# gchq/annchor

Hardware: AMD Instinct MI355X
Metric: knn_graph_builds_per_s (1 / Annchor.fit() wall-clock; BASELINE: k-NN graph build time + recall@k) (higher is better)
Workload: dtype int32 bit-vectors (Levenshtein) + f64 (bounds/regression/selection); 1 GPU; load_strings Levenshtein N=1600 n_anchors=15 k=25 p_work=0.12 niters=2; parallelism=one GPU

## Files before the change

annchor_amd/csrc/ctx.hip:

```cpp
#include <cstdarg>
#include <cmath>
#include <cstdlib>

#include "common.h"
#include <algorithm>
#include <chrono>
#include <mutex>

static std::string g_create_err;
void ann_stream_release(annchor_ctx *c);
void ann_enemies_release(annchor_ctx *c);
void ann_draw_forget(annchor_ctx *c);
void ann_comm_release(annchor_ctx *c);
hipError_t ann_comm_guarded_sync(annchor_ctx *c, hipStream_t stream, const char *where);

const char *ann_set_err(annchor_ctx *c, const char *fmt, ...)
{
    char buf[1024];
    va_list ap;
    va_start(ap, fmt);
    vsnprintf(buf, sizeof buf, fmt, ap);
    va_end(ap);
    if (c && c->comm_aborted && c->err.rfind("collective timed out", 0) == 0) return c->err.c_str();
    if (c) c->err = buf; else g_create_err = buf;
// ... 179 lines not shown
        ANN_CHECK_HIP(c, hipMemcpyAsync(dst, slot, bytes, hipMemcpyHostToDevice, c->stream));
        ANN_CHECK_HIP(c, hipEventRecord(c->pin_ev[sl], c->stream));
        c->pin_busy[sl] = true;
        return ANNCHOR_OK;
    }
    ANN_CHECK_HIP(c, hipMemcpyAsync(dst, src, bytes, hipMemcpyHostToDevice, c->stream));
    ANN_CHECK_HIP(c, ann_sync(c, __func__));
    return ANNCHOR_OK;
}

hipError_t ann_sync(annchor_ctx *c, const char *where)
{
    static const bool trace = getenv("ANNCHOR_SYNC_TRACE") != nullptr;
    static const bool timing = getenv("ANNCHOR_SYNC_TIMING") != nullptr;
    if (trace) fprintf(stderr, "sync %s\n", where);
    const long long t_in = timing ? ann_now_ns() : 0;
    if (c->idle_gen_n > c->idle_gen_done) {
        c->idle_gen_done = std::min(c->idle_gen_n, c->idle_gen_done + c->idle_gen_chunk);
        (void)ann_legacy_generate_upto(c->idle_gen_seed, c->idle_gen_n, c->idle_gen_done);
    }
    const long long t_w = timing ? ann_now_ns() : 0;
    if (c->side_pending) (void)ann_side_join(c);
    const hipError_t rc = c->comm ? ann_comm_guarded_sync(c, c->stream, where) : hipStreamSynchronize(c->stream);
    if (timing) fprintf(stderr, "T wait %s %lld %lld %lld\n", where, t_in, t_w, ann_now_ns());
    if (c->lev_ap_probe_epoch) ann_lev_ap_probe(c);
    return rc;
}

extern "C" int annchor_legacy_generate_at_next_wait(annchor_ctx *c, uint32_t seed, int64_t ndraws, int64_t chunk)
{
    if (!c || ndraws < 0) return ANNCHOR_EINVAL;
    c->idle_gen_seed = seed;
    c->idle_gen_n = ndraws;
    c->idle_gen_done = 0;
    c->idle_gen_chunk = chunk > 0 ? chunk : ndraws;
    return ANNCHOR_OK;
}

int ann_d2h(annchor_ctx *c, void *dst, const void *src, size_t bytes)
{
    if (bytes == 0) return ANNCHOR_OK;
    if (c->pin && bytes <= annchor_ctx::PIN_DL_BYTES) {
        unsigned char *slot = c->pin + (size_t)annchor_ctx::PIN_SLOTS * annchor_ctx::PIN_SLOT_BYTES;
        ANN_CHECK_HIP(c, hipMemcpyAsync(slot, src, bytes, hipMemcpyDeviceToHost, c->stream));
        ANN_CHECK_HIP(c, ann_sync(c, __func__));
        memcpy(dst, slot, bytes);
        return ANNCHOR_OK;
    }
    ANN_CHECK_HIP(c, hipMemcpyAsync(dst, src, bytes, hipMemcpyDeviceToHost, c->stream));
    ANN_CHECK_HIP(c, ann_sync(c, __func__));
    return ANNCHOR_OK;
}

int ann_d2h2(annchor_ctx *c, void *dst1, const void *src1, size_t bytes1, void *dst2, const void *src2, size_t bytes2)
{
    const size_t off2 = (bytes1 + 63) & ~(size_t)63;
    if (c->pin && off2 + bytes2 <= annchor_ctx::PIN_DL_BYTES) {
        unsigned char *slot = c->pin + (size_t)annchor_ctx::PIN_SLOTS * annchor_ctx::PIN_SLOT_BYTES;
        ANN_CHECK_HIP(c, hipMemcpyAsync(slot, src1, bytes1, hipMemcpyDeviceToHost, c->stream));
        ANN_CHECK_HIP(c, hipMemcpyAsync(slot + off2, src2, bytes2, hipMemcpyDeviceToHost, c->stream));
        ANN_CHECK_HIP(c, ann_sync(c, __func__));
        memcpy(dst1, slot, bytes1);
        memcpy(dst2, slot + off2, bytes2);
        return ANNCHOR_OK;
    }
    ANN_TRY(ann_d2h(c, dst1, src1, bytes1));
    return ann_d2h(c, dst2, src2, bytes2);
}

int ann_d2h_then(annchor_ctx *c, void *dst, const void *src, size_t bytes, int (*then)(annchor_ctx *))
{
    if (!c->pin || bytes > annchor_ctx::PIN_DL_BYTES) {
        ANN_TRY(ann_d2h(c, dst, src, bytes));
        return then(c);
    }
    if (!c->dl_ev) ANN_CHECK_HIP(c, hipEventCreate(&c->dl_ev));
    unsigned char *slot = c->pin + (size_t)annchor_ctx::PIN_SLOTS * annchor_ctx::PIN_SLOT_BYTES;
    ANN_CHECK_HIP(c, hipMemcpyAsync(slot, src, bytes, hipMemcpyDeviceToHost, c->stream));
    ANN_CHECK_HIP(c, hipEventRecord(c->dl_ev, c->stream));
    const int rc = then(c);
    static const bool trace = getenv("ANNCHOR_SYNC_TRACE") != nullptr;
    static const bool timing = getenv("ANNCHOR_SYNC_TIMING") != nullptr;
    if (trace) fprintf(stderr, "sync %s\n", __func__);
    const long long t_w = timing ? ann_now_ns() : 0;
    ANN_CHECK_HIP(c, hipEventSynchronize(c->dl_ev));
    if (timing) fprintf(stderr, "T wait %s %lld %lld %lld\n", __func__, t_w, t_w, ann_now_ns());
    memcpy(dst, slot, bytes);
    return rc;
}

int ann_prof_entry(annchor_ctx *c, const char *name)
{
    for (size_t i = 0; i < c->prof.size(); ++i)
        if (c->prof[i].name == name || strcmp(c->prof[i].name, name) == 0) return (int)i;
    ProfEntry e;
    e.name = name;
    c->prof.push_back(e);
    return (int)c->prof.size() - 1;
}

static void prof_drain(annchor_ctx *c)
{
    for (auto &p : c->pending) {
        float ms = 0;
        if (hipEventSynchronize(p.b) == hipSuccess && hipEventElapsedTime(&ms, p.a, p.b) == hipSuccess)
            c->prof[p.entry].ms += ms;
        c->ev_pool.push_back(p.a);
        c->ev_pool.push_back(p.b);
    }
    c->pending.clear();
}

ProfScope::ProfScope(annchor_ctx *ctx, const char *name, double alg_bytes) : c(ctx)
{
    if (!c->prof_on) return;
    if (c->prof_mode == 2) {
        const size_t n = strlen(name);
        if (n < 6 || strcmp(name + n - 6, "_pairs") != 0) return;
    }
    entry = ann_prof_entry(c, name);
    c->prof[entry].launches += 1;
    c->prof[entry].alg_bytes += alg_bytes;
    if (entry == c->prof_group_entry) { entry = -1; return; }
    auto get = [&](hipEvent_t *e) {
        if (!c->ev_pool.empty()) { *e = c->ev_pool.back(); c->ev_pool.pop_back(); return true; }
        return hipEventCreate(e) == hipSuccess;
    };
    if (!get(&a) || !get(&b)) { entry = -1; return; }
    (void)hipEventRecord(a, c->stream);
}

ProfGroup::ProfGroup(annchor_ctx *ctx, const char *name) : c(ctx)
{
    if (!c->prof_on || c->prof_group_entry >= 0) return;
    if (c->prof_mode == 2) {
        const size_t n = strlen(name);
        if (n < 6 || strcmp(name + n - 6, "_pairs") != 0) return;
    }
    entry = ann_prof_entry(c, name);
    auto get = [&](hipEvent_t *e) {
        if (!c->ev_pool.empty()) { *e = c->ev_pool.back(); c->ev_pool.pop_back(); return true; }
        return hipEventCreate(e) == hipSuccess;
    };
    if (!get(&a) || !get(&b)) { entry = -1; return; }
    (void)hipEventRecord(a, c->stream);
    c->prof_group_entry = entry;
}

ProfGroup::~ProfGroup()
{
    if (entry < 0) return;
    (void)hipEventRecord(b, c->stream);
    c->pending.push_back({entry, a, b});
    c->prof_group_entry = -1;
}

ProfScope::~ProfScope()
{
    if (entry < 0) return;
    (void)hipEventRecord(b, c->stream);
    c->pending.push_back({entry, a, b});
    if (c->pending.size() > 4096) prof_drain(c);
}

extern "C" int annchor_prof_enable(annchor_ctx *c, int32_t on)
{
    if (!c) return ANNCHOR_EINVAL;
    c->prof_on = on != 0;
    c->prof_mode = on;
    return ANNCHOR_OK;
// ... 1073 lines not shown
```

annchor_amd/csrc/locality.hip:

```cpp
#include "common.h"

template <int NW> __global__ void k_sid(const double *__restrict__ Dt, int64_t nx, int na, int locality, uint64_t *__restrict__ sid,
                                        int32_t *__restrict__ cA)
{
    int64_t i = (int64_t)blockIdx.x * blockDim.x + threadIdx.x;
    if (i >= nx) return;
    Sid<NW> mask = sid_zero<NW>();
    int first = 0;
    for (int r = 0; r < locality; ++r) {
        double best = INFINITY;
        int ba = -1;
        for (int a = 0; a < na; ++a) {
            if ((mask.w[NW == 1 ? 0 : a >> 6] >> (a & 63)) & 1ull) continue;
            double v = Dt[(size_t)a * nx + i];
            if (ba < 0 || v < best) { best = v; ba = a; }
        }
        if (ba < 0) break;
        if (r == 0) first = ba;
#pragma unroll
        for (int w = 0; w < NW; ++w)
            if (w == (ba >> 6)) mask.w[w] |= 1ull << (ba & 63);
    }
#pragma unroll
    for (int w = 0; w < NW; ++w) sid[i * NW + w] = mask.w[w];
    cA[i] = first;
}

#define LOC_THREADS 256
template <int NW>
__global__ __launch_bounds__(LOC_THREADS) void k_loc_thresh(const uint64_t *__restrict__ sid, int64_t nx, int loc_thresh,
                                                           int loc_min, int32_t *__restrict__ thr)
{
    __shared__ uint32_t hist[ANN_MASK_ANCHORS + 1];
    for (int t = threadIdx.x; t < ANN_MASK_ANCHORS + 1; t += blockDim.x) hist[t] = 0;
    __syncthreads();
    const int64_t i = blockIdx.x;
    const Sid<NW> mi = sid_ld<NW>(sid, i);
    for (int64_t j = threadIdx.x; j < nx; j += blockDim.x) atomicAdd(&hist[sid_common<NW>(mi, sid_ld<NW>(sid, j))], 1u);
    __syncthreads();
    if (threadIdx.x == 0) {
        int64_t lm = loc_min < nx - 1 ? loc_min : nx - 1;
        int64_t cum = 0;
        int v = ANN_MASK_ANCHORS;
        for (; v >= 0; --v) {
            cum += hist[v];
            if (cum >= lm + 1) break;
        }
        if (v < 0) v = 0;
        thr[i] = v < loc_thresh ? v : loc_thresh;
    }
}

template <int T, int NW>
__global__ __launch_bounds__(LOC_THREADS) void k_loc_thresh_small(const uint64_t *__restrict__ sid, int64_t nx, int loc_min, int32_t *__restrict__ thr)
{
    __shared__ uint32_t part[LOC_THREADS / 64][T];
    const int64_t i = blockIdx.x;
    const Sid<NW> mi = sid_ld<NW>(sid, i);
    uint32_t c[T];
#pragma unroll
    for (int t = 0; t < T; ++t) c[t] = 0;
    for (int64_t j0 = threadIdx.x; j0 < nx; j0 += 4 * LOC_THREADS) {
        Sid<NW> mj[4];
#pragma unroll
        for (int e = 0; e < 4; ++e) mj[e] = sid_ld<NW>(sid, min(j0 + e * LOC_THREADS, nx - 1));
#pragma unroll
        for (int e = 0; e < 4; ++e) {
            const int cc = j0 + e * LOC_THREADS < nx ? sid_common<NW>(mi, mj[e]) : 0;
#pragma unroll
            for (int t = 0; t < T; ++t) c[t] += cc > t;
        }
    }
#pragma unroll
    for (int t = 0; t < T; ++t) {
#pragma unroll
        for (int off = 32; off > 0; off >>= 1) c[t] += __shfl_xor(c[t], off);
    }
    if ((threadIdx.x & 63) == 0)
#pragma unroll
        for (int t = 0; t < T; ++t) part[threadIdx.x >> 6][t] = c[t];
    __syncthreads();
    if (threadIdx.x == 0) {
        const int64_t lm = loc_min < nx - 1 ? loc_min : nx - 1;
        int v = 0;
#pragma unroll
        for (int t = 0; t < T; ++t) {
            uint32_t g = 0;
            for (int w = 0; w < LOC_THREADS / 64; ++w) g += part[w][t];
            if ((int64_t)g >= lm + 1) v = t + 1;
        }
        thr[i] = v;
    }
}

template <int NW>
__global__ __launch_bounds__(256) void k_keep_bits(const uint64_t *__restrict__ sid, const int32_t *__restrict__ thr, int64_t nx, int kw,
                                                  uint64_t *__restrict__ K)
{
    const int lane = threadIdx.x & 63;
    const int64_t wave_global = ((int64_t)blockIdx.x * blockDim.x + threadIdx.x) >> 6;
    const int64_t wave_count = ((int64_t)gridDim.x * blockDim.x) >> 6;
    const int64_t items = nx * kw;
    const int64_t per = (items + wave_count - 1) / wave_count;
    const int64_t t0 = wave_global * per, t1 = min(t0 + per, items);
    for (int64_t t = t0; t < t1; ++t) {
        const int64_t i = t / kw;
        const int w = (int)(t - i * kw);
        const Sid<NW> mi = sid_ld<NW>(sid, i);
        const int ti = thr[i];
        const int64_t j = (int64_t)w * 64 + lane;
        bool keep = false;
        if (j < nx && j != i) {
            const int cc = sid_common<NW>(mi, sid_ld<NW>(sid, j));
            const int tj = thr[j];
            keep = cc >= (ti < tj ? ti : tj);
        }
        const unsigned long long bits = __ballot(keep);
        if (lane == 0) K[t] = bits;
    }
}

template <int NW>
__global__ __launch_bounds__(256) void k_keep_bits_cols(const uint64_t *__restrict__ sid, const int32_t *__restrict__ thr, int64_t nx, int kw,
                                                       uint64_t *__restrict__ K)
{
    const int lane = threadIdx.x & 63;
    const int wave = __builtin_amdgcn_readfirstlane((int)(threadIdx.x >> 6));
    const int64_t task = (int64_t)blockIdx.x * 4 + wave;
    const int64_t rb = task / kw;
    const int w = (int)(task - rb * kw);
    if (rb * 64 >= nx) return;
    const int64_t i0 = rb * 64, i_base = min(i0, nx - 64);
    const int64_t j = (int64_t)w * 64 + lane;
    const bool jv = j < nx;
    const Sid<NW> mj = jv ? sid_ld<NW>(sid, j) : sid_zero<NW>();
    const int tj = jv ? thr[j] : 0;
    int r_lo = 0, r_hi = 0;
#pragma unroll 16
    for (int r = 0; r < 64; ++r) {
        const int64_t i = i_base + r;
        const Sid<NW> mi = sid_ld<NW>(sid, i);
        const int ti = thr[i];
        const int cc = sid_common<NW>(mi, mj);
        const bool keep = jv && j != i && cc >= (ti < tj ? ti : tj);
        const unsigned long long bits = __ballot(keep);
        r_lo = lane == r ? (int)(uint32_t)bits : r_lo;
        r_hi = lane == r ? (int)(uint32_t)(bits >> 32) : r_hi;
    }
    const int64_t i = i_base + lane;
    if (i >= i0) K[i * kw + w] = ((uint64_t)(uint32_t)r_hi << 32) | (uint32_t)r_lo;
}

__global__ void k_sid_wide(const double *__restrict__ Dt, int64_t nx, int na, int L, int nw, int kw, uint64_t *__restrict__ sid,
                           uint16_t *__restrict__ sidl, uint64_t *__restrict__ sidm, int32_t *__restrict__ cA)
{
    const int64_t i = (int64_t)blockIdx.x * blockDim.x + threadIdx.x;
    if (i >= nx) return;
    double pv = -INFINITY;
    int pa = -1, first = 0;
    for (int r = 0; r < L; ++r) {
        double best = INFINITY;
        int ba = -1;
        for (int a = 0; a < na; ++a) {
            const double v = Dt[(size_t)a * nx + i];
            const bool after = v > pv || (v == pv && a > pa);
            if (after && (ba < 0 || v < best)) { best = v; ba = a; }
        }
        if (ba < 0) {
            for (; r < L; ++r) sidl[i * L + r] = 0xffff;
            break;
        }
        if (r == 0) first = ba;
        sidl[i * L + r] = (uint16_t)ba;
        sid[i * nw + (ba >> 6)] |= 1ull << (ba & 63);
        atomicOr(reinterpret_cast<unsigned long long *>(sidm) + (size_t)ba * kw + (i >> 6), 1ull << (i & 63));
        pv = best; pa = ba;
    }
    cA[i] = first;
}

template <int T>
__global__ __launch_bounds__(LOC_THREADS) void k_loc_thresh_small_wide(const uint16_t *__restrict__ sidl, const uint64_t *__restrict__ sidm,
                                                                      int L, int na, int kw, int64_t nx, int loc_min, int32_t *__restrict__ thr)
{
    __shared__ uint32_t part[LOC_THREADS / 64][T];
    const int64_t i = blockIdx.x;
    uint32_t c[T];
#pragma unroll
    for (int t = 0; t < T; ++t) c[t] = 0;
    for (int w = threadIdx.x; w < kw; w += LOC_THREADS) {
        uint64_t ge[T + 1];
        ge[0] = ~0ull;
#pragma unroll
        for (int k = 1; k <= T; ++k) ge[k] = 0ull;
        for (int r = 0; r < L; ++r) {
            const int a = sidl[i * L + r];
            const uint64_t m = a < na ? sidm[(size_t)a * kw + w] : 0ull;
#pragma unroll
            for (int k = T; k >= 1; --k) ge[k] |= ge[k - 1] & m;
        }
#pragma unroll
// ... 255 lines not shown
    } else {
        const int64_t t = blockIdx.x;
        jb = (int)((2.0 * nb + 1.0 - sqrt((2.0 * nb + 1.0) * (2.0 * nb + 1.0) - 8.0 * (double)t)) * 0.5);
        while ((int64_t)jb * nb - (int64_t)jb * (jb - 1) / 2 > t) --jb;
        while ((int64_t)(jb + 1) * nb - (int64_t)(jb + 1) * jb / 2 <= t) ++jb;
        ib = jb + (int)(t - ((int64_t)jb * nb - (int64_t)jb * (jb - 1) / 2));
    }
    const int lane = threadIdx.x & 63, wave = threadIdx.x >> 6;
    const int64_t i_r = (int64_t)ib * 64 + lane;
#pragma unroll 4
    for (int q = 0; q < 16; ++q) {
        const int64_t j = (int64_t)jb * 64 + wave * 16 + q;
        int32_t pos = 0;
        if (j < nx) {
            const uint64_t bits = K[j * kw + ib];
            if (i_r > j && ((bits >> lane) & 1ull))
                pos = (int32_t)(rowstart[j] + ((int64_t)pref[j * kw + ib] + __popcll(bits & ((1ull << lane) - 1ull)) - low[j]));
        }
        tp[wave * 16 + q][lane] = pos;
    }
    __syncthreads();
    const int64_t j_w = (int64_t)jb * 64 + lane;
    uint32_t cb_lo = 0, cb_hi = 0, cd_lo = 0, cd_hi = 0;
    {
        const int64_t i = (int64_t)ib * 64 + wave * 16 + (lane & 15);
        if (i < nx) {
            const uint64_t bits = K[i * kw + jb];
            const int64_t dst0 = Iptr[i] + (int64_t)pref[i * kw + jb];
            cb_lo = (uint32_t)bits; cb_hi = (uint32_t)(bits >> 32);
            cd_lo = (uint32_t)dst0; cd_hi = (uint32_t)((uint64_t)dst0 >> 32);
        }
    }
#pragma unroll
    for (int q = 0; q < 16; ++q) {
        const int il = wave * 16 + q;
        const int64_t i = (int64_t)ib * 64 + il;
        const uint64_t bits = ((uint64_t)(uint32_t)__builtin_amdgcn_readlane((int)cb_hi, q) << 32) | (uint32_t)__builtin_amdgcn_readlane((int)cb_lo, q);
        if (j_w < i && ((bits >> lane) & 1ull)) {
            const int64_t dst0 = (int64_t)(((uint64_t)(uint32_t)__builtin_amdgcn_readlane((int)cd_hi, q) << 32) | (uint32_t)__builtin_amdgcn_readlane((int)cd_lo, q));
            ann_store(Iidx + dst0 + __popcll(bits & ((1ull << lane) - 1ull)), tp[lane][il], stream);
        }
    }
}

__global__ void k_min_i32(const int32_t *__restrict__ v, int64_t n, int32_t *__restrict__ out)
{
    int m = 0x7fffffff;
    for (int64_t t = threadIdx.x; t < n; t += blockDim.x) m = min(m, v[t]);
#pragma unroll
    for (int off = 32; off > 0; off >>= 1) m = min(m, __shfl_xor(m, off));
    __shared__ int s[16];
    if ((threadIdx.x & 63) == 0) s[threadIdx.x >> 6] = m;
    __syncthreads();
    if (threadIdx.x == 0) {
        for (int w = 1; w < (int)(blockDim.x >> 6); ++w) m = min(m, s[w]);
        out[0] = m;
        out[1] = 0; out[2] = 0; out[3] = 0;
    }
}

__global__ __launch_bounds__(256) void k_count_anchor_pairs(const int32_t *__restrict__ A, int nA, const int32_t *__restrict__ anchorRank,
                                                           int64_t nx, const uint64_t *__restrict__ K, int kw,
                                                           unsigned long long *__restrict__ out)
{
    const int64_t t = (int64_t)blockIdx.x * blockDim.x + threadIdx.x;
    bool hit = false;
    if (t < (int64_t)nA * nx) {
        const int r = (int)(t / nx);
        const int64_t a = A[r], o = t % nx;
        if (anchorRank[a] == r && a != o && !(anchorRank[o] >= 0 && o < a)) {
            const int64_t i = a < o ? a : o, j = a < o ? o : a;
            hit = (K[i * kw + (j >> 6)] >> (j & 63)) & 1ull;
        }
    }
    const unsigned long long m = __ballot(hit);
    __shared__ uint32_t s;
    if (threadIdx.x == 0) s = 0;
    __syncthreads();
    if ((threadIdx.x & 63) == 0 && m) atomicAdd(&s, (uint32_t)__popcll(m));
    __syncthreads();
    if (threadIdx.x == 0 && s) atomicAdd(out, (unsigned long long)s);
}

static int wide_sets(annchor_ctx *c, int locality)
{
    const int64_t nx = c->nx;
    const int nw = c->sid_nw, kw = (int)((nx + 63) / 64);
    c->sid_L = locality;
    ANN_TRY(ann_reserve(c, c->sidl, sizeof(uint16_t) * (size_t)nx * locality));
    ANN_TRY(ann_reserve(c, c->sidm, sizeof(uint64_t) * (size_t)c->na * kw));
    ANN_CHECK_HIP(c, hipMemsetAsync(c->sid.p, 0, sizeof(uint64_t) * (size_t)nx * nw, c->stream));
    ANN_CHECK_HIP(c, hipMemsetAsync(c->sidm.p, 0, sizeof(uint64_t) * (size_t)c->na * kw, c->stream));
    k_sid_wide<<<ann_blocks(nx, 256), 256, 0, c->stream>>>(c->Dt.as<double>(), nx, c->na, locality, nw, kw, c->sid.as<uint64_t>(),
                                                          c->sidl.as<uint16_t>(), c->sidm.as<uint64_t>(), c->cA.as<int32_t>());
    return ANNCHOR_OK;
}

static int wide_keep_bitmap(annchor_ctx *c, int loc_thresh, int loc_min, int kw)
{
    const int64_t nx = c->nx;
    const int L = c->sid_L, na = c->na;
    const uint16_t *sidl = c->sidl.as<uint16_t>();
    const uint64_t *sidm = c->sidm.as<uint64_t>();
    static const bool hist_form = getenv("ANNCHOR_LOC_THRESH_HIST") != nullptr;
    if (loc_thresh >= 1 && loc_thresh <= 8 && !hist_form) {
        switch (loc_thresh) {
#define LTW_CASE(T) case T: k_loc_thresh_small_wide<T><<<(int)nx, LOC_THREADS, 0, c->stream>>>(sidl, sidm, L, na, kw, nx, loc_min, c->thr.as<int32_t>()); break;
            LTW_CASE(1) LTW_CASE(2) LTW_CASE(3) LTW_CASE(4) LTW_CASE(5) LTW_CASE(6) LTW_CASE(7) LTW_CASE(8)
#undef LTW_CASE
        }
    } else
        k_loc_thresh_wide<<<(int)nx, LOC_THREADS, sizeof(uint32_t) * (size_t)(L + 1), c->stream>>>(sidl, sidm, L, na, kw, nx, loc_thresh,
                                                                                                 loc_min, c->thr.as<int32_t>());
    const unsigned grid = (unsigned)((((nx + 63) / 64) * kw + 3) / 4);
    if (loc_thresh >= 1 && loc_thresh <= 8) {
        switch (loc_thresh) {
#define KBP_CASE(T) case T: k_keep_bits_wide_planes<T><<<grid, 256, 0, c->stream>>>(sidl, sidm, L, na, c->thr.as<int32_t>(), nx, kw, c->Kbits.as<uint64_t>()); break;
            KBP_CASE(1) KBP_CASE(2) KBP_CASE(3) KBP_CASE(4) KBP_CASE(5) KBP_CASE(6) KBP_CASE(7) KBP_CASE(8)
#undef KBP_CASE
        }
        return ANNCHOR_OK;
    }
    switch (L) {
#define KBW_CASE(LC) case LC: k_keep_bits_wide<LC><<<grid, 256, 0, c->stream>>>(sidl, sidm, L, na, c->thr.as<int32_t>(), nx, kw, c->Kbits.as<uint64_t>()); break;
        KBW_CASE(1) KBW_CASE(2) KBW_CASE(3) KBW_CASE(4) KBW_CASE(5) KBW_CASE(6) KBW_CASE(7) KBW_CASE(8)
#undef KBW_CASE
    default: k_keep_bits_wide<0><<<grid, 256, 0, c->stream>>>(sidl, sidm, L, na, c->thr.as<int32_t>(), nx, kw, c->Kbits.as<uint64_t>());
    }
    return ANNCHOR_OK;
}

extern "C" int annchor_build_locality(annchor_ctx *c, int32_t locality, int32_t loc_thresh, int32_t loc_min,
                                      int64_t *n_pairs, int64_t *min_row_len)
{
    if (!c || !n_pairs || !min_row_len) return ANNCHOR_EINVAL;
    ANN_REQUIRE(c, c->na > 0, ANNCHOR_EINVAL, "anchors not set");
    ANN_REQUIRE(c, locality >= 1, ANNCHOR_EINVAL, "locality must be >= 1");
    ANN_CHECK_HIP(c, hipSetDevice(c->device));
    const int64_t nx = c->nx;
    const int kw = (int)((nx + 63) / 64);
    ANN_REQUIRE(c, (double)nx * kw * 12.0 < 64e9, ANNCHOR_ELIMIT,
                "nx=%lld is too large for the pair-list form (use the streamed form)", (long long)nx);
    if (locality > c->na) locality = c->na;
    const int nw = c->sid_nw = ann_sid_words(c->na);
    const bool wide = ann_sid_wide(c->na);
    ANN_TRY(ann_reserve(c, c->sid, sizeof(uint64_t) * (size_t)nx * nw));
    ANN_TRY(ann_reserve(c, c->cA, sizeof(int32_t) * (size_t)nx));
    ANN_TRY(ann_reserve(c, c->thr, sizeof(int32_t) * (size_t)nx));
    ANN_TRY(ann_reserve(c, c->Kbits, sizeof(uint64_t) * (size_t)nx * kw));
    ANN_TRY(ann_reserve(c, c->Kpref, sizeof(uint32_t) * (size_t)nx * kw));
    ANN_TRY(ann_reserve(c, c->deg, sizeof(int32_t) * (size_t)nx));
    ANN_TRY(ann_reserve(c, c->low, sizeof(int32_t) * (size_t)nx));
    ANN_TRY(ann_reserve(c, c->tmp1, sizeof(int32_t) * (size_t)nx));
    ANN_TRY(ann_reserve(c, c->rowstart, sizeof(int64_t) * (size_t)(nx + 1)));
    ANN_TRY(ann_reserve(c, c->Iptr, sizeof(int64_t) * (size_t)(nx + 1)));
    ANN_TRY(ann_reserve(c, c->tmp2, sizeof(int32_t) * 4));
    ANN_CHECK_HIP(c, hipEventRecord(c->call_a, c->stream));
    {
        ProfScope ps(c, "locality_sid", (double)nx * (c->na * 8.0 + 12));
        if (wide)
            ANN_TRY(wide_sets(c, locality));
        else {
#define SID_CALL(NW) k_sid<NW><<<ann_blocks(nx, 256), 256, 0, c->stream>>>(c->Dt.as<double>(), nx, c->na, locality, c->sid.as<uint64_t>(), c->cA.as<int32_t>())
        ANN_SID_DISPATCH(nw, SID_CALL);
#undef SID_CALL
        }
    }
    {
        ProfScope ps(c, "locality_keep_bitmap", (double)nx * kw * 12.0);
        if (wide)
            ANN_TRY(wide_keep_bitmap(c, loc_thresh, loc_min, kw));
        else {
        static const bool hist_form = getenv("ANNCHOR_LOC_THRESH_HIST") != nullptr;
        if (loc_thresh >= 1 && loc_thresh <= 8 && !hist_form) {
            switch (loc_thresh) {
#define LT_NW(NW) k_loc_thresh_small<LT_T, NW><<<(int)nx, LOC_THREADS, 0, c->stream>>>(c->sid.as<uint64_t>(), nx, loc_min, c->thr.as<int32_t>())
#define LT_CASE(T) case T: { constexpr int LT_T = T; ANN_SID_DISPATCH(nw, LT_NW); } break;
                LT_CASE(1) LT_CASE(2) LT_CASE(3) LT_CASE(4) LT_CASE(5) LT_CASE(6) LT_CASE(7) LT_CASE(8)
#undef LT_CASE
#undef LT_NW
            }
        } else {
#define LTH_CALL(NW) k_loc_thresh<NW><<<(int)nx, LOC_THREADS, 0, c->stream>>>(c->sid.as<uint64_t>(), nx, loc_thresh, loc_min, c->thr.as<int32_t>())
            ANN_SID_DISPATCH(nw, LTH_CALL);
#undef LTH_CALL
        }
        static const long long cols_min = getenv("ANNCHOR_KEEP_COLS_MIN") ? atoll(getenv("ANNCHOR_KEEP_COLS_MIN")) : (1ll << 20);
        if (nx >= 64 && nx * kw >= cols_min) {
#define KBC_CALL(NW) k_keep_bits_cols<NW><<<(unsigned)((((nx + 63) / 64) * kw + 3) / 4), 256, 0, c->stream>>>(c->sid.as<uint64_t>(), c->thr.as<int32_t>(), nx, kw, c->Kbits.as<uint64_t>())
            ANN_SID_DISPATCH(nw, KBC_CALL);
#undef KBC_CALL
        } else {
#define KB_CALL(NW) k_keep_bits<NW><<<(int)std::min<int64_t>(ann_blocks(nx * kw * 64, 256), (int64_t)c->prop.multiProcessorCount * 32), 256, 0, c->stream>>>(c->sid.as<uint64_t>(), c->thr.as<int32_t>(), nx, kw, c->Kbits.as<uint64_t>())
            ANN_SID_DISPATCH(nw, KB_CALL);
#undef KB_CALL
        }
        }
        k_row_prefix<<<(int)nx, LOC_THREADS, 0, c->stream>>>(c->Kbits.as<uint64_t>(), nx, kw, c->Kpref.as<uint32_t>(),
                                                            c->deg.as<int32_t>(), c->low.as<int32_t>(),
                                                            c->tmp1.as<int32_t>());
        k_min_i32<<<1, 1024, 0, c->stream>>>(c->deg.as<int32_t>(), nx, c->tmp2.as<int32_t>());
        if (c->nA > 0 && c->anchorRank.p)
            k_count_anchor_pairs<<<ann_blocks((int64_t)c->nA * nx, 256), 256, 0, c->stream>>>(
                c->A.as<int32_t>(), c->nA, c->anchorRank.as<int32_t>(), nx, c->Kbits.as<uint64_t>(), kw,
                reinterpret_cast<unsigned long long *>(c->tmp2.as<int32_t>() + 2));
    }
    ANN_TRY(ann_exclusive_scan_i32_to_i64(c, c->tmp1.as<int32_t>(), c->rowstart.as<int64_t>(), nx));
    ANN_TRY(ann_exclusive_scan_i32_to_i64(c, c->deg.as<int32_t>(), c->Iptr.as<int64_t>(), nx));
    int64_t n = 0;
    struct { int32_t mn, pad; long long anchor_pairs; } st = {0, 0, 0};
    ANN_TRY(ann_d2h2(c, &n, c->rowstart.as<int64_t>() + nx, sizeof n, &st, c->tmp2.p, sizeof st));
    const int32_t mn = st.mn;
    c->n_unc_after_features = (c->nA > 0 && c->anchorRank.p) ? n - st.anchor_pairs : -1;
    ANN_REQUIRE(c, n < (1ll << 30), ANNCHOR_ELIMIT,
                "%lld candidate pairs exceed the pair-list limit of 2^30 (int32 positions): raise loc_thresh / lower locality", (long long)n);
    if (n > (1ll << 27)) {
        size_t fr = 0, tot = 0;
        ANN_CHECK_HIP(c, hipMemGetInfo(&fr, &tot));
        int64_t parked = 0;
        (void)annchor_parked_bytes(c->device, &parked);
        const double have = (double)fr + (double)parked + (double)c->ij.cap + (double)c->Iidx.cap + (double)c->lb.cap + (double)c->ub.cap + (double)c->dad.cap + (double)c->RA.cap + (double)c->prob.cap;
        ANN_REQUIRE(c, (double)n * 130.0 <= have, ANNCHOR_ELIMIT,
                    "%lld candidate pairs need ~%.0f GB of device memory, %.0f GB are free: raise loc_thresh / lower locality",
                    (long long)n, (double)n * 130.0 / 1e9, have / 1e9);
    }
    ANN_TRY(ann_reserve(c, c->ij, sizeof(int2) * (size_t)n));
    ANN_TRY(ann_reserve(c, c->Iidx, sizeof(int32_t) * 2 * (size_t)n));
    {
        ProfScope ps(c, "locality_emit_pairs", (double)n * 16 + (double)nx * kw * 12.0);
        static const long long tiled_min = getenv("ANNCHOR_EMIT_TILED_MIN") ? atoll(getenv("ANNCHOR_EMIT_TILED_MIN")) : 0;
        const int stream_hint = n >= ANN_STREAM_MIN_PAIRS, tiled = n >= tiled_min;
        static const long long run_min = getenv("ANNCHOR_EMIT_RUN_MIN") ? atoll(getenv("ANNCHOR_EMIT_RUN_MIN")) : (1ll << 20);
        if (tiled && nx * kw >= run_min)
            k_emit_rows_run<<<(int)std::min<int64_t>(ann_blocks(nx * kw, 256), (int64_t)c->prop.multiProcessorCount * 32), 256, 0, c->stream>>>(
                c->Kbits.as<uint64_t>(), c->Kpref.as<uint32_t>(), nx, kw, c->low.as<int32_t>(), c->rowstart.as<int64_t>(),
                c->Iptr.as<int64_t>(), c->ij.as<int2>(), c->Iidx.as<int32_t>(), stream_hint);
        else
        k_emit_pairs<<<(int)std::min<int64_t>(ann_blocks(nx * kw * 64, 256), (int64_t)c->prop.multiProcessorCount * 64), 256, 0, c->stream>>>(
            c->Kbits.as<uint64_t>(), c->Kpref.as<uint32_t>(), nx, kw, c->low.as<int32_t>(), c->rowstart.as<int64_t>(),
            c->Iptr.as<int64_t>(), c->ij.as<int2>(), c->Iidx.as<int32_t>(), stream_hint, tiled);
        if (tiled) {
            const int64_t S = (kw + EC_SUPER - 1) / EC_SUPER;
            static const int super_min = getenv("ANNCHOR_EMIT_SUPER_MIN") ? atoi(getenv("ANNCHOR_EMIT_SUPER_MIN")) : 4 * EC_SUPER;
            const int supertiles = kw >= super_min;
            const int64_t grid = supertiles ? ((S * (S + 1) / 2 + 7) / 8) * 8 * EC_SUPER * EC_SUPER : (int64_t)kw * (kw + 1) / 2;
            k_emit_cols<<<(unsigned)grid, 256, 0, c->stream>>>(
                c->Kbits.as<uint64_t>(), c->Kpref.as<uint32_t>(), kw, c->low.as<int32_t>(), c->rowstart.as<int64_t>(),
                c->Iptr.as<int64_t>(), nx, c->Iidx.as<int32_t>(), stream_hint, supertiles);
        }
    }
    ANN_CHECK_HIP(c, hipEventRecord(c->call_b, c->stream));
    c->call_timed = true;
    ANN_CHECK_HIP(c, hipGetLastError());
    c->n = n;
    c->have_bitmap = true;
    c->have_features = c->have_RA = false; c->sel_prepared = false; ann_mask_changed(c);
    *n_pairs = n;
    *min_row_len = mn;
    return ANNCHOR_OK;
}

template <int NW>
__global__ __launch_bounds__(LOC_THREADS) void k_qloc_count(const uint64_t *__restrict__ sid, int64_t nxb, int loc_thresh,
                                                           int32_t *__restrict__ cnt)
{
    __shared__ uint32_t acc;
    if (threadIdx.x == 0) acc = 0;
    __syncthreads();
    const int64_t q = nxb + blockIdx.x;
    const Sid<NW> mq = sid_ld<NW>(sid, q);
    uint32_t s = 0;
    for (int64_t i = threadIdx.x; i < nxb; i += blockDim.x) s += sid_common<NW>(mq, sid_ld<NW>(sid, i)) >= loc_thresh;
    if (s) atomicAdd(&acc, s);
    __syncthreads();
    if (threadIdx.x == 0) cnt[q] = (int32_t)acc;
}

template <int NW>
__global__ __launch_bounds__(LOC_THREADS) void k_qloc_emit(const uint64_t *__restrict__ sid, int64_t nxb, int loc_thresh,
                                                          const int64_t *__restrict__ Iptr, int2 *__restrict__ ij,
                                                          int32_t *__restrict__ Iidx)
{
    __shared__ uint32_t wsum[LOC_THREADS / 64];
    __shared__ uint32_t run_s;
    const int64_t q = nxb + blockIdx.x;
    const Sid<NW> mq = sid_ld<NW>(sid, q);
    const int lane = threadIdx.x & 63, wave = threadIdx.x >> 6;
    if (threadIdx.x == 0) run_s = 0;
    __syncthreads();
    const int64_t base = Iptr[q];
    for (int64_t b0 = 0; b0 < nxb; b0 += LOC_THREADS) {
        const int64_t i = b0 + threadIdx.x;
        const uint32_t f = (i < nxb && sid_common<NW>(mq, sid_ld<NW>(sid, min(i, nxb - 1))) >= loc_thresh) ? 1u : 0u;
        const unsigned long long m = __ballot(f);
        if (lane == 0) wsum[wave] = (uint32_t)__popcll(m);
        __syncthreads();
        uint32_t pre = run_s;
        for (int w = 0; w < wave; ++w) pre += wsum[w];
        if (f) {
            const int64_t pos = base + pre + (uint32_t)__popcll(m & ((1ull << lane) - 1ull));
            ij[pos] = make_int2((int)i, (int)q);
            Iidx[pos] = (int32_t)pos;
        }
        __syncthreads();
        if (threadIdx.x == 0) run_s += wsum[0] + wsum[1] + wsum[2] + wsum[3];
        __syncthreads();
    }
}

__global__ __launch_bounds__(LOC_THREADS) void k_qloc_count_wide(const uint16_t *__restrict__ sidl, const uint64_t *__restrict__ sidm, int L,
                                                                int na, int kw, int64_t nxb, int loc_thresh, int32_t *__restrict__ cnt)
{
    __shared__ uint32_t acc;
    if (threadIdx.x == 0) acc = 0;
    __syncthreads();
    const int64_t q = nxb + blockIdx.x;
    const int wave = __builtin_amdgcn_readfirstlane((int)(threadIdx.x >> 6));
    uint32_t s = 0;
    for (int64_t w = wave; w * 64 < nxb; w += LOC_THREADS / 64) {
        const int cc = sidm_common(sidl, sidm, L, na, kw, q, w);
        s += w * 64 + (threadIdx.x & 63) < nxb && cc >= loc_thresh;
    }
    if (s) atomicAdd(&acc, s);
    __syncthreads();
    if (threadIdx.x == 0) cnt[q] = (int32_t)acc;
}

__global__ __launch_bounds__(LOC_THREADS) void k_qloc_emit_wide(const uint16_t *__restrict__ sidl, const uint64_t *__restrict__ sidm, int L,
                                                               int na, int kw, int64_t nxb, int loc_thresh, const int64_t *__restrict__ Iptr,
                                                               int2 *__restrict__ ij, int32_t *__restrict__ Iidx)
{
    __shared__ uint32_t wsum[LOC_THREADS / 64];
// ... 95 lines not shown
```

Baseline: 395.0 graphs/s.

## Fuse locality build kernels and emit pair lists before host readback

Adds a register-resident anchor-set kernel for single-word masks, fuses keep-bit computation with the per-row prefix/degree pass, and replaces min/anchor-count/two scans with one single-block finisher kernel for small N. For small problems it reserves worst-case pair buffers and enqueues the pair emission before waiting on the count readback, overlapping the host sync with GPU work. It also piggybacks idle legacy generation and a probe onto the d2h wait. This trades extra memory reservation and single-block serial work for fewer launches and syncs.

```diff
diff --git a/annchor_amd/csrc/ctx.hip b/annchor_amd/csrc/ctx.hip
--- a/annchor_amd/csrc/ctx.hip
+++ b/annchor_amd/csrc/ctx.hip
@@ -285,10 +285,16 @@
     static const bool trace = getenv("ANNCHOR_SYNC_TRACE") != nullptr;
     static const bool timing = getenv("ANNCHOR_SYNC_TIMING") != nullptr;
     if (trace) fprintf(stderr, "sync %s\n", __func__);
+    const long long t_in = timing ? ann_now_ns() : 0;
+    if (c->idle_gen_n > c->idle_gen_done) {
+        c->idle_gen_done = std::min(c->idle_gen_n, c->idle_gen_done + c->idle_gen_chunk);
+        (void)ann_legacy_generate_upto(c->idle_gen_seed, c->idle_gen_n, c->idle_gen_done);
+    }
     const long long t_w = timing ? ann_now_ns() : 0;
     ANN_CHECK_HIP(c, hipEventSynchronize(c->dl_ev));
-    if (timing) fprintf(stderr, "T wait %s %lld %lld %lld\n", __func__, t_w, t_w, ann_now_ns());
+    if (timing) fprintf(stderr, "T wait %s %lld %lld %lld\n", __func__, t_in, t_w, ann_now_ns());
     memcpy(dst, slot, bytes);
+    if (c->lev_ap_probe_epoch) ann_lev_ap_probe(c);
     return rc;
 }
 
diff --git a/annchor_amd/csrc/locality.hip b/annchor_amd/csrc/locality.hip
--- a/annchor_amd/csrc/locality.hip
+++ b/annchor_amd/csrc/locality.hip
@@ -26,6 +26,30 @@
     cA[i] = first;
 }
 
+template <int NAC> __global__ __launch_bounds__(64) void k_sid_regs(const double *__restrict__ Dt, int64_t nx, int na, int locality,
+                                                                   uint64_t *__restrict__ sid, int32_t *__restrict__ cA)
+{
+    const int64_t i = (int64_t)blockIdx.x * blockDim.x + threadIdx.x;
+    if (i >= nx) return;
+    double v[NAC];
+#pragma unroll
+    for (int a = 0; a < NAC; ++a) v[a] = Dt[(size_t)min(a, na - 1) * nx + i];
+    uint64_t mask = 0ull;
+    int first = 0;
+    for (int r = 0; r < locality; ++r) {
+        double best = INFINITY;
+        int ba = -1;
+#pragma unroll
+        for (int a = 0; a < NAC; ++a)
+            if (a < na && !((mask >> a) & 1ull) && (ba < 0 || v[a] < best)) { best = v[a]; ba = a; }
+        if (ba < 0) break;
+        if (r == 0) first = ba;
+        mask |= 1ull << ba;
+    }
+    sid[i] = mask;
+    cA[i] = first;
+}
+
 #define LOC_THREADS 256
 template <int NW>
 __global__ __launch_bounds__(LOC_THREADS) void k_loc_thresh(const uint64_t *__restrict__ sid, int64_t nx, int loc_thresh,
@@ -93,21 +117,20 @@
     }
 }
 
+#define KEEP_ROW_MAX_KW 4096
 template <int NW>
-__global__ __launch_bounds__(256) void k_keep_bits(const uint64_t *__restrict__ sid, const int32_t *__restrict__ thr, int64_t nx, int kw,
-                                                  uint64_t *__restrict__ K)
-{
-    const int lane = threadIdx.x & 63;
-    const int64_t wave_global = ((int64_t)blockIdx.x * blockDim.x + threadIdx.x) >> 6;
-    const int64_t wave_count = ((int64_t)gridDim.x * blockDim.x) >> 6;
-    const int64_t items = nx * kw;
-    const int64_t per = (items + wave_count - 1) / wave_count;
-    const int64_t t0 = wave_global * per, t1 = min(t0 + per, items);
-    for (int64_t t = t0; t < t1; ++t) {
-        const int64_t i = t / kw;
-        const int w = (int)(t - i * kw);
-        const Sid<NW> mi = sid_ld<NW>(sid, i);
-        const int ti = thr[i];
+__global__ __launch_bounds__(LOC_THREADS) void k_keep_bits_row(const uint64_t *__restrict__ sid, const int32_t *__restrict__ thr, int64_t nx, int kw,
+                                                         uint64_t *__restrict__ K, uint32_t *__restrict__ pref, int32_t *__restrict__ deg,
+                                                         int32_t *__restrict__ low, int32_t *__restrict__ up)
+{
+    extern __shared__ uint64_t rowbits[];
+    __shared__ uint32_t wsum[LOC_THREADS / 64];
+    __shared__ uint32_t carry_s, low_s;
+    const int64_t i = blockIdx.x;
+    const int lane = threadIdx.x & 63, wave = threadIdx.x >> 6;
+    const Sid<NW> mi = sid_ld<NW>(sid, i);
+    const int ti = thr[i];
+    for (int w = wave; w < kw; w += LOC_THREADS / 64) {
         const int64_t j = (int64_t)w * 64 + lane;
         bool keep = false;
         if (j < nx && j != i) {
@@ -116,7 +139,36 @@
             keep = cc >= (ti < tj ? ti : tj);
         }
         const unsigned long long bits = __ballot(keep);
-        if (lane == 0) K[t] = bits;
+        if (lane == 0) { rowbits[w] = bits; K[i * kw + w] = bits; }
+    }
+    if (threadIdx.x == 0) carry_s = 0;
+    __syncthreads();
+    const int wi = (int)(i >> 6);
+    for (int base = 0; base < kw; base += LOC_THREADS) {
+        const int w = base + threadIdx.x;
+        const uint64_t bw = w < kw ? rowbits[w] : 0ull;
+        const uint32_t v = (uint32_t)__popcll(bw);
+        uint32_t inc = v;
+#pragma unroll
+        for (int off = 1; off < 64; off <<= 1) {
+            uint32_t o = __shfl_up(inc, off);
+            if (lane >= off) inc += o;
+        }
+        if (lane == 63) wsum[wave] = inc;
+        __syncthreads();
+        uint32_t b = carry_s;
+        for (int ww = 0; ww < wave; ++ww) b += wsum[ww];
+        if (w < kw) pref[i * kw + w] = b + inc - v;
+        if (w == wi) low_s = b + inc - v + (uint32_t)__popcll(bw & ((1ull << (i & 63)) - 1ull));
+        __syncthreads();
+        if (threadIdx.x == LOC_THREADS - 1) carry_s = b + inc;
+        __syncthreads();
+    }
+    if (threadIdx.x == 0) {
+        const uint32_t d = carry_s, l = low_s;
+        deg[i] = (int32_t)d;
+        low[i] = (int32_t)l;
+        up[i] = (int32_t)(d - l);
     }
 }
 
@@ -538,6 +590,92 @@
     if (threadIdx.x == 0 && s) atomicAdd(out, (unsigned long long)s);
 }
 
+#define FIN_THREADS 1024
+#define FIN_ITEMS 8
+#define FIN_SLOTS 16
+#define FIN_MAX_ANCHOR_ITEMS (1 << 17)
+__global__ __launch_bounds__(FIN_THREADS) void k_loc_finish(const int32_t *__restrict__ up, const int32_t *__restrict__ deg, int nx,
+                                                           const int32_t *__restrict__ A, int nA, const int32_t *__restrict__ anchorRank,
+                                                           const uint64_t *__restrict__ K, int kw, int64_t *__restrict__ rowstart,
+                                                           int64_t *__restrict__ Iptr, int32_t *__restrict__ out)
+{
+    __shared__ int64_t ws_up[FIN_THREADS / 64], ws_deg[FIN_THREADS / 64];
+    __shared__ int32_t ws_min[FIN_THREADS / 64];
+    __shared__ uint32_t ws_cnt[FIN_THREADS / 64];
+    const int lane = threadIdx.x & 63, wave = threadIdx.x >> 6;
+    const int base = (int)threadIdx.x * FIN_ITEMS;
+    int32_t u[FIN_ITEMS], d[FIN_ITEMS];
+#pragma unroll
+    for (int k = 0; k < FIN_ITEMS; ++k) { u[k] = ann_ldc(up, base + k, nx); d[k] = ann_ldc(deg, base + k, nx); }
+    int64_t su = 0, sd = 0;
+    int32_t m = 0x7fffffff;
+#pragma unroll
+    for (int k = 0; k < FIN_ITEMS; ++k) {
+        if (base + k >= nx) { u[k] = 0; d[k] = 0; }
+        else m = min(m, d[k]);
+        su += u[k]; sd += d[k];
+    }
+    const uint32_t *__restrict__ K32 = reinterpret_cast<const uint32_t *>(K);
+    uint32_t cnt = 0;
+    for (int r0 = 0; r0 < nA; r0 += FIN_SLOTS) {
+        int a[FIN_SLOTS];
+        bool live[FIN_SLOTS];
+#pragma unroll
+        for (int e = 0; e < FIN_SLOTS; ++e) a[e] = A[min(r0 + e, nA - 1)];
+#pragma unroll
+        for (int e = 0; e < FIN_SLOTS; ++e) live[e] = r0 + e < nA && anchorRank[a[e]] == r0 + e;
+        for (int o0 = 0; o0 < nx; o0 += 2 * FIN_THREADS) {
+            int o[2], ro[2];
+            uint32_t kb[2][FIN_SLOTS];
+#pragma unroll
+            for (int h = 0; h < 2; ++h) {
+                o[h] = min(o0 + h * FIN_THREADS + (int)threadIdx.x, nx - 1);
+                ro[h] = anchorRank[o[h]];
+#pragma unroll
+                for (int e = 0; e < FIN_SLOTS; ++e)
+                    kb[h][e] = K32[(int64_t)a[e] * kw * 2 + (o[h] >> 5)] >> (o[h] & 31);
+            }
+#pragma unroll
+            for (int h = 0; h < 2; ++h)
+#pragma unroll
+                for (int e = 0; e < FIN_SLOTS; ++e)
+                    cnt += o0 + h * FIN_THREADS + (int)threadIdx.x < nx && live[e] && a[e] != o[h] && !(ro[h] >= 0 && o[h] < a[e]) &&
+                           (kb[h][e] & 1u);
+        }
+    }
+    int64_t iu = su, id = sd;
+#pragma unroll
+    for (int off = 1; off < 64; off <<= 1) {
+        const int64_t ou = __shfl_up(iu, off), od = __shfl_up(id, off);
+        if (lane >= off) { iu += ou; id += od; }
+    }
+#pragma unroll
+    for (int off = 32; off > 0; off >>= 1) { m = min(m, __shfl_xor(m, off)); cnt += __shfl_xor(cnt, off); }
+    if (lane == 63) { ws_up[wave] = iu; ws_deg[wave] = id; }
+    if (lane == 0) { ws_min[wave] = m; ws_cnt[wave] = cnt; }
+    __syncthreads();
+    int64_t pu = 0, pd = 0, tu = 0, td = 0;
+    for (int w = 0; w < FIN_THREADS / 64; ++w) {
+        const int64_t xu = ws_up[w], xd = ws_deg[w];
+        if (w < wave) { pu += xu; pd += xd; }
+        tu += xu; td += xd;
+    }
+    int64_t eu = pu + iu - su, ed = pd + id - sd;
+#pragma unroll
+    for (int k = 0; k < FIN_ITEMS; ++k) {
+        if (base + k < nx) { rowstart[base + k] = eu; Iptr[base + k] = ed; }
+        eu += u[k]; ed += d[k];
+    }
+    if (threadIdx.x == 0) {
+        unsigned long long c = 0;
+        for (int w = 0; w < FIN_THREADS / 64; ++w) { m = min(m, ws_min[w]); c += ws_cnt[w]; }
+        rowstart[nx] = tu; Iptr[nx] = td;
+        out[0] = m; out[1] = 0;
+        *reinterpret_cast<unsigned long long *>(out + 2) = c;
+        *reinterpret_cast<long long *>(out + 4) = (long long)tu;
+    }
+}
+
 static int wide_sets(annchor_ctx *c, int locality)
 {
     const int64_t nx = c->nx;
@@ -585,6 +723,35 @@
     }
     return ANNCHOR_OK;
 }
+
+static int emit_lists(annchor_ctx *c, int stream_hint, int tiled, double list_bytes)
+{
+    const int64_t nx = c->nx;
+    const int kw = (int)((nx + 63) / 64);
+    ProfScope ps(c, "locality_emit_pairs", list_bytes + (double)nx * kw * 12.0);
+    static const long long run_min = getenv("ANNCHOR_EMIT_RUN_MIN") ? atoll(getenv("ANNCHOR_EMIT_RUN_MIN")) : (1ll << 20);
+    if (tiled && nx * kw >= run_min)
+        k_emit_rows_run<<<(int)std::min<int64_t>(ann_blocks(nx * kw, 256), (int64_t)c->prop.multiProcessorCount * 32), 256, 0, c->stream>>>(
+            c->Kbits.as<uint64_t>(), c->Kpref.as<uint32_t>(), nx, kw, c->low.as<int32_t>(), c->rowstart.as<int64_t>(),
+            c->Iptr.as<int64_t>(), c->ij.as<int2>(), c->Iidx.as<int32_t>(), stream_hint);
+    else
+        k_emit_pairs<<<(int)std::min<int64_t>(ann_blocks(nx * kw * 64, 256), (int64_t)c->prop.multiProcessorCount * 64), 256, 0, c->stream>>>(
+            c->Kbits.as<uint64_t>(), c->Kpref.as<uint32_t>(), nx, kw, c->low.as<int32_t>(), c->rowstart.as<int64_t>(),
+            c->Iptr.as<int64_t>(), c->ij.as<int2>(), c->Iidx.as<int32_t>(), stream_hint, tiled);
+    if (tiled) {
+        const int64_t S = (kw + EC_SUPER - 1) / EC_SUPER;
+        static const int super_min = getenv("ANNCHOR_EMIT_SUPER_MIN") ? atoi(getenv("ANNCHOR_EMIT_SUPER_MIN")) : 4 * EC_SUPER;
+        const int supertiles = kw >= super_min;
+        const int64_t grid = supertiles ? ((S * (S + 1) / 2 + 7) / 8) * 8 * EC_SUPER * EC_SUPER : (int64_t)kw * (kw + 1) / 2;
+        k_emit_cols<<<(unsigned)grid, 256, 0, c->stream>>>(
+            c->Kbits.as<uint64_t>(), c->Kpref.as<uint32_t>(), kw, c->low.as<int32_t>(), c->rowstart.as<int64_t>(),
+            c->Iptr.as<int64_t>(), nx, c->Iidx.as<int32_t>(), stream_hint, supertiles);
+    }
+    return ANNCHOR_OK;
+}
+
+#define EMIT_EARLY_MAX_BYTES (256ll << 20)
+static int emit_lists_early(annchor_ctx *c) { return emit_lists(c, 0, 1, 0.0); }
 
 extern "C" int annchor_build_locality(annchor_ctx *c, int32_t locality, int32_t loc_thresh, int32_t loc_min,
                                       int64_t *n_pairs, int64_t *min_row_len)
@@ -610,13 +777,22 @@
     ANN_TRY(ann_reserve(c, c->tmp1, sizeof(int32_t) * (size_t)nx));
     ANN_TRY(ann_reserve(c, c->rowstart, sizeof(int64_t) * (size_t)(nx + 1)));
     ANN_TRY(ann_reserve(c, c->Iptr, sizeof(int64_t) * (size_t)(nx + 1)));
-    ANN_TRY(ann_reserve(c, c->tmp2, sizeof(int32_t) * 4));
+    ANN_TRY(ann_reserve(c, c->tmp2, sizeof(int32_t) * 8));
     ANN_CHECK_HIP(c, hipEventRecord(c->call_a, c->stream));
+    const int nA_count = (c->nA > 0 && c->anchorRank.p) ? c->nA : 0;
+    const bool finisher = nx <= FIN_THREADS * FIN_ITEMS && (int64_t)nA_count * nx <= FIN_MAX_ANCHOR_ITEMS;
+    bool rows_done = false;
     {
         ProfScope ps(c, "locality_sid", (double)nx * (c->na * 8.0 + 12));
         if (wide)
             ANN_TRY(wide_sets(c, locality));
-        else {
+        else if (nw == 1) {
+#define SIDR_CALL(NAC) k_sid_regs<NAC><<<ann_blocks(nx, 64), 64, 0, c->stream>>>(c->Dt.as<double>(), nx, c->na, locality, c->sid.as<uint64_t>(), c->cA.as<int32_t>())
+            if (c->na <= 16) SIDR_CALL(16);
+            else if (c->na <= 32) SIDR_CALL(32);
+            else SIDR_CALL(64);
+#undef SIDR_CALL
+        } else {
 #define SID_CALL(NW) k_sid<NW><<<ann_blocks(nx, 256), 256, 0, c->stream>>>(c->Dt.as<double>(), nx, c->na, locality, c->sid.as<uint64_t>(), c->cA.as<int32_t>())
         ANN_SID_DISPATCH(nw, SID_CALL);
 #undef SID_CALL
@@ -642,30 +818,55 @@
 #undef LTH_CALL
         }
         static const long long cols_min = getenv("ANNCHOR_KEEP_COLS_MIN") ? atoll(getenv("ANNCHOR_KEEP_COLS_MIN")) : (1ll << 20);
-        if (nx >= 64 && nx * kw >= cols_min) {
+        if (nx >= 64 && (nx * kw >= cols_min || kw > KEEP_ROW_MAX_KW)) {
 #define KBC_CALL(NW) k_keep_bits_cols<NW><<<(unsigned)((((nx + 63) / 64) * kw + 3) / 4), 256, 0, c->stream>>>(c->sid.as<uint64_t>(), c->thr.as<int32_t>(), nx, kw, c->Kbits.as<uint64_t>())
             ANN_SID_DISPATCH(nw, KBC_CALL);
 #undef KBC_CALL
         } else {
-#define KB_CALL(NW) k_keep_bits<NW><<<(int)std::min<int64_t>(ann_blocks(nx * kw * 64, 256), (int64_t)c->prop.multiProcessorCount * 32), 256, 0, c->stream>>>(c->sid.as<uint64_t>(), c->thr.as<int32_t>(), nx, kw, c->Kbits.as<uint64_t>())
-            ANN_SID_DISPATCH(nw, KB_CALL);
-#undef KB_CALL
-        }
-        }
-        k_row_prefix<<<(int)nx, LOC_THREADS, 0, c->stream>>>(c->Kbits.as<uint64_t>(), nx, kw, c->Kpref.as<uint32_t>(),
-                                                            c->deg.as<int32_t>(), c->low.as<int32_t>(),
-                                                            c->tmp1.as<int32_t>());
-        k_min_i32<<<1, 1024, 0, c->stream>>>(c->deg.as<int32_t>(), nx, c->tmp2.as<int32_t>());
-        if (c->nA > 0 && c->anchorRank.p)
-            k_count_anchor_pairs<<<ann_blocks((int64_t)c->nA * nx, 256), 256, 0, c->stream>>>(
-                c->A.as<int32_t>(), c->nA, c->anchorRank.as<int32_t>(), nx, c->Kbits.as<uint64_t>(), kw,
-                reinterpret_cast<unsigned long long *>(c->tmp2.as<int32_t>() + 2));
-    }
-    ANN_TRY(ann_exclusive_scan_i32_to_i64(c, c->tmp1.as<int32_t>(), c->rowstart.as<int64_t>(), nx));
-    ANN_TRY(ann_exclusive_scan_i32_to_i64(c, c->deg.as<int32_t>(), c->Iptr.as<int64_t>(), nx));
+#define KR_CALL(NW) k_keep_bits_row<NW><<<(int)nx, LOC_THREADS, sizeof(uint64_t) * (size_t)kw, c->stream>>>(c->sid.as<uint64_t>(), c->thr.as<int32_t>(), nx, kw, c->Kbits.as<uint64_t>(), c->Kpref.as<uint32_t>(), c->deg.as<int32_t>(), c->low.as<int32_t>(), c->tmp1.as<int32_t>())
+            ANN_SID_DISPATCH(nw, KR_CALL);
+#undef KR_CALL
+            rows_done = true;
+        }
+        }
+        if (!rows_done)
+            k_row_prefix<<<(int)nx, LOC_THREADS, 0, c->stream>>>(c->Kbits.as<uint64_t>(), nx, kw, c->Kpref.as<uint32_t>(),
+                                                                c->deg.as<int32_t>(), c->low.as<int32_t>(),
+                                                                c->tmp1.as<int32_t>());
+        if (finisher)
+            k_loc_finish<<<1, FIN_THREADS, 0, c->stream>>>(c->tmp1.as<int32_t>(), c->deg.as<int32_t>(), (int)nx, c->A.as<int32_t>(), nA_count,
+                                                          c->anchorRank.as<int32_t>(), c->Kbits.as<uint64_t>(), kw,
+                                                          c->rowstart.as<int64_t>(), c->Iptr.as<int64_t>(), c->tmp2.as<int32_t>());
+        else {
+            k_min_i32<<<1, 1024, 0, c->stream>>>(c->deg.as<int32_t>(), nx, c->tmp2.as<int32_t>());
+            if (nA_count > 0)
+                k_count_anchor_pairs<<<ann_blocks((int64_t)c->nA * nx, 256), 256, 0, c->stream>>>(
+                    c->A.as<int32_t>(), c->nA, c->anchorRank.as<int32_t>(), nx, c->Kbits.as<uint64_t>(), kw,
+                    reinterpret_cast<unsigned long long *>(c->tmp2.as<int32_t>() + 2));
+        }
+    }
+    if (!finisher) {
+        ANN_TRY(ann_exclusive_scan_i32_to_i64(c, c->tmp1.as<int32_t>(), c->rowstart.as<int64_t>(), nx));
+        ANN_TRY(ann_exclusive_scan_i32_to_i64(c, c->deg.as<int32_t>(), c->Iptr.as<int64_t>(), nx));
+    }
+    static const long long tiled_min = getenv("ANNCHOR_EMIT_TILED_MIN") ? atoll(getenv("ANNCHOR_EMIT_TILED_MIN")) : 0;
+    const int64_t n_bound = nx * (nx - 1) / 2;
+    const bool early = finisher && tiled_min <= 0 && n_bound * 16 <= EMIT_EARLY_MAX_BYTES && n_bound < ANN_STREAM_MIN_PAIRS;
     int64_t n = 0;
-    struct { int32_t mn, pad; long long anchor_pairs; } st = {0, 0, 0};
-    ANN_TRY(ann_d2h2(c, &n, c->rowstart.as<int64_t>() + nx, sizeof n, &st, c->tmp2.p, sizeof st));
+    struct { int32_t mn, pad; long long anchor_pairs; long long n; } st = {0, 0, 0, 0};
+    if (early) {
+        ANN_TRY(ann_reserve(c, c->ij, sizeof(int2) * (size_t)n_bound));
+        ANN_TRY(ann_reserve(c, c->Iidx, sizeof(int32_t) * 2 * (size_t)n_bound));
+        ANN_TRY(ann_d2h_then(c, &st, c->tmp2.p, sizeof st, emit_lists_early));
+        n = st.n;
+        ANN_REQUIRE(c, n <= n_bound && n < ANN_STREAM_MIN_PAIRS, ANNCHOR_ELIMIT,
+                    "%lld candidate pairs from %lld points", (long long)n, (long long)nx);
+        if (c->prof_on && c->prof_mode != 2) c->prof[ann_prof_entry(c, "locality_emit_pairs")].alg_bytes += (double)n * 16;
+    } else if (finisher) {
+        ANN_TRY(ann_d2h(c, &st, c->tmp2.p, sizeof st));
+        n = st.n;
+    } else
+        ANN_TRY(ann_d2h2(c, &n, c->rowstart.as<int64_t>() + nx, sizeof n, &st, c->tmp2.p, 16));
     const int32_t mn = st.mn;
     c->n_unc_after_features = (c->nA > 0 && c->anchorRank.p) ? n - st.anchor_pairs : -1;
     ANN_REQUIRE(c, n < (1ll << 30), ANNCHOR_ELIMIT,
@@ -680,30 +881,10 @@
                     "%lld candidate pairs need ~%.0f GB of device memory, %.0f GB are free: raise loc_thresh / lower locality",
                     (long long)n, (double)n * 130.0 / 1e9, have / 1e9);
     }
-    ANN_TRY(ann_reserve(c, c->ij, sizeof(int2) * (size_t)n));
-    ANN_TRY(ann_reserve(c, c->Iidx, sizeof(int32_t) * 2 * (size_t)n));
-    {
-        ProfScope ps(c, "locality_emit_pairs", (double)n * 16 + (double)nx * kw * 12.0);
-        static const long long tiled_min = getenv("ANNCHOR_EMIT_TILED_MIN") ? atoll(getenv("ANNCHOR_EMIT_TILED_MIN")) : 0;
-        const int stream_hint = n >= ANN_STREAM_MIN_PAIRS, tiled = n >= tiled_min;
-        static const long long run_min = getenv("ANNCHOR_EMIT_RUN_MIN") ? atoll(getenv("ANNCHOR_EMIT_RUN_MIN")) : (1ll << 20);
-        if (tiled && nx * kw >= run_min)
-            k_emit_rows_run<<<(int)std::min<int64_t>(ann_blocks(nx * kw, 256), (int64_t)c->prop.multiProcessorCount * 32), 256, 0, c->stream>>>(
-                c->Kbits.as<uint64_t>(), c->Kpref.as<uint32_t>(), nx, kw, c->low.as<int32_t>(), c->rowstart.as<int64_t>(),
-                c->Iptr.as<int64_t>(), c->ij.as<int2>(), c->Iidx.as<int32_t>(), stream_hint);
-        else
-        k_emit_pairs<<<(int)std::min<int64_t>(ann_blocks(nx * kw * 64, 256), (int64_t)c->prop.multiProcessorCount * 64), 256, 0, c->stream>>>(
-            c->Kbits.as<uint64_t>(), c->Kpref.as<uint32_t>(), nx, kw, c->low.as<int32_t>(), c->rowstart.as<int64_t>(),
-            c->Iptr.as<int64_t>(), c->ij.as<int2>(), c->Iidx.as<int32_t>(), stream_hint, tiled);
-        if (tiled) {
-            const int64_t S = (kw + EC_SUPER - 1) / EC_SUPER;
-            static const int super_min = getenv("ANNCHOR_EMIT_SUPER_MIN") ? atoi(getenv("ANNCHOR_EMIT_SUPER_MIN")) : 4 * EC_SUPER;
-            const int supertiles = kw >= super_min;
-            const int64_t grid = supertiles ? ((S * (S + 1) / 2 + 7) / 8) * 8 * EC_SUPER * EC_SUPER : (int64_t)kw * (kw + 1) / 2;
-            k_emit_cols<<<(unsigned)grid, 256, 0, c->stream>>>(
-                c->Kbits.as<uint64_t>(), c->Kpref.as<uint32_t>(), kw, c->low.as<int32_t>(), c->rowstart.as<int64_t>(),
-                c->Iptr.as<int64_t>(), nx, c->Iidx.as<int32_t>(), stream_hint, supertiles);
-        }
+    if (!early) {
+        ANN_TRY(ann_reserve(c, c->ij, sizeof(int2) * (size_t)n));
+        ANN_TRY(ann_reserve(c, c->Iidx, sizeof(int32_t) * 2 * (size_t)n));
+        ANN_TRY(emit_lists(c, n >= ANN_STREAM_MIN_PAIRS, n >= tiled_min, (double)n * 16));
     }
     ANN_CHECK_HIP(c, hipEventRecord(c->call_b, c->stream));
     c->call_timed = true;
```

After: 398.5 graphs/s (median of 2 runs). About the same (+0.9%).
